# tesseract-robotics/trajopt

Measured on NVIDIA H100. Metric: converged trajectories/sec (7-DOF x 30 wp, batch 1024), higher is better.
Workload: dtype f64

## Files before the change

### trajopt_b200/csrc/kernels.h

```cpp
#pragma once
#include "device_types.cuh"

namespace tb200 {
struct EvalExtra;
struct SolveCtl;
using SolveKernelFn = void (*)(DevProblem, EvalExtra, SolveCtl);
using EvalKernelFn = void (*)(DevProblem, EvalExtra, int, const double*);
SolveKernelFn solve_kernel_for(int D, bool pair_rows, bool sing);
EvalKernelFn eval_kernel_for(int D, bool sing);
int eval_debug_prof(unsigned long long* out, int reset);
constexpr int kQpProfSlots = 32;
int qp_debug_prof(unsigned long long* out, int reset);
}
```

### trajopt_b200/csrc/qp_cta_kernel.cuh

```cuda
#pragma once
#include "device_types.cuh"
#include "joint_terms.cuh"

namespace tb200 {

#ifdef TB200_PROFILE
static __device__ unsigned long long g_prof[32];
#define PROF_T0() const long long prof_t0_ = clock64()
#define PROF_ADD(slot) do { if (q.tid == 0) atomicAdd(&g_prof[slot], (unsigned long long)(clock64() - prof_t0_)); } while (0)
#define PROF_COUNT(slot) do { if (q.tid == 0) atomicAdd(&g_prof[slot], 1ull); } while (0)
#define PROF_ADD2(slot, slot2) do { if (q.tid == 0) { const unsigned long long d_ = clock64() - prof_t0_; \
    atomicAdd(&g_prof[slot], d_); atomicAdd(&g_prof[slot2], d_); } } while (0)
#else
#define PROF_T0()
#define PROF_ADD(slot)
#define PROF_COUNT(slot)
#define PROF_ADD2(slot, slot2)
#endif
#if defined(TB200_PROFILE) && defined(TB200_PROFILE_CHECK)
#define PROF_CHK_T0() long long pc_ = clock64()
#define PROF_CHK(slot) do { const long long n_ = clock64(); if (q.tid == 0) atomicAdd(&g_prof[slot], (unsigned long long)(n_ - pc_)); pc_ = n_; } while (0)
#else
#define PROF_CHK_T0()
#define PROF_CHK(slot)
#endif

constexpr int kQpThreads = 256;
constexpr int kQpThreadsC = 256;
constexpr double kOsqpInf = 1e30;
constexpr double kMinScaling = 1e-4, kMaxScaling = 1e4;
constexpr double kVerifyTol = 1e-9;
constexpr int kVerifyRounds = 3;
constexpr double kRhoMin = 1e-6, kRhoMax = 1e6, kRhoTol = 1e-4, kRhoEqOverIneq = 1e3;
enum { QPS_UNSOLVED = 0, QPS_SOLVED = 1, QPS_SOLVED_INACC = 2, QPS_PINF = 3, QPS_PINF_INACC = 4, QPS_DINF = 5,
       QPS_DINF_INACC = 6, QPS_MAXITER = 7, QPS_NONCVX = 8 };

__device__ __forceinline__ double limit_scaling(double v) {
  v = v < kMinScaling ? 1.0 : v;
  return v > kMaxScaling ? kMaxScaling : v;
}

struct QpSmem {
  int SA, SLM, SU, beta, x, zb, yb, v1, w, qs, lbs, ubs, Dz, v2, Pb, tmp, red, colptr, colent, rints, rows, total, row_cap;
  int factor_smem, pband_smem;
  int pinv;
};

struct PinvPlan {
  int ok;
  int Ns, nS;
  int PR;
  int ZS, HO;
  int WS;
  int SS;
  int zo, wo, so;
  int total;
};
__host__ __device__ inline PinvPlan pinv_plan(int M, int nb) {
  PinvPlan pl;
  pl.Ns = M / 4;
  pl.nS = pl.Ns * nb;
  pl.PR = (M - pl.Ns) * nb;
  const int Np = M * nb, blk = nb * nb;
  pl.ok = (nb % 2 == 0) && nb <= 14 && pl.Ns <= 3 && pl.PR + 2 * pl.nS <= 256;
  pl.ZS = Np + ((4 - Np % 16) + 16) % 16;
  pl.HO = ((Np / 2 + 6) / 16) * 16 + 2;
  if (pl.HO > Np) pl.HO = Np;
  pl.WS = 2 * nb + 2;
  pl.SS = pl.nS + (pl.nS & 1);
  const int fA = (M * blk + 15) & ~15, fL = fA + 8, fU = (M * blk + 1) & ~1;
  const int zn = pl.nS * pl.ZS;
  pl.zo = 0;
  pl.wo = ((zn > fA + fL + fU ? zn : fA + fL + fU) + 15) & ~15;
  pl.so = pl.wo + ((pl.PR * pl.WS + 1) & ~1);
  pl.total = pl.so + pl.nS * pl.SS;
  return pl;
}
constexpr int kQpSmemBudget = 28800;
__host__ __device__ inline int qp_block_count(int N, int nb) { return (N + nb - 1) / nb; }
__host__ __device__ inline int qp_even(int v) { return (v + 1) & ~1; }
__host__ __device__ inline int qp_factor_doubles(int N, int nb) { return 3 * qp_even(qp_block_count(N, nb) * nb * nb); }
__host__ __device__ inline size_t qp_cta_global_doubles(int N, int nb) {
  const PinvPlan pl = pinv_plan(qp_block_count(N, nb), nb);
  return static_cast<size_t>(qp_factor_doubles(N, nb)) + static_cast<size_t>(pl.nS) * pl.ZS;
}
__host__ __device__ inline QpSmem qp_smem_layout(int N, int nb, int row_stride, int CN, int max_rows, bool factor_global) {
  const int M = qp_block_count(N, nb), Np = M * nb, blk = nb * nb;
  QpSmem s;
  int o = 0;
  s.beta = o; o += qp_even(Np);
  s.x = o;    o += qp_even(Np);
  s.zb = o;   o += qp_even(Np);
  s.yb = o;   o += qp_even(Np);
  s.v1 = o;   o += qp_even(Np);
  s.w = o;    o += qp_even(Np);
  s.qs = o;   o += qp_even(Np);
  s.lbs = o;  o += qp_even(Np);
  s.ubs = o;  o += qp_even(Np);
  s.Dz = o;   o += qp_even(Np);
  s.v2 = o;   o += qp_even(Np);
// ... 103 lines not shown
    double v = vals[k];
    if ((SUM_MASK >> k) & 1u) {
#pragma unroll
      for (int off = 16; off > 0; off >>= 1) v += __shfl_xor_sync(0xffffffffu, v, off);
    } else {
      v = warp_max_norm(v);
    }
    vals[k] = v;
  }
  if (lane == 0) {
#pragma unroll
    for (int k = 0; k < NQ; ++k) red[k * 8 + wid] = vals[k];
  }
  __syncthreads();
#pragma unroll
  for (int k = 0; k < NQ; ++k) {
    if ((SUM_MASK >> k) & 1u) {
      double acc = red[k * 8];
#pragma unroll
      for (int w = 1; w < kQpThreads / 32; ++w) acc += red[k * 8 + w];
      vals[k] = acc;
    } else {
      vals[k] = warp_max_norm(red[k * 8 + (lane & 7)]);
    }
  }
  __syncthreads();
}

struct SysW {
  bool polish;
  double sig, rho_aux;
#ifdef TB200_PROFILE
  int prof_kind = 0;
#endif
};

__device__ __forceinline__ int row_var(const int* I, int k) {
  return I[RI_BASE] + min(k, I[RI_CNT] - 1) * I[RI_STRIDE];
}

template <int NB>
__device__ __forceinline__ void load_row(double (&a)[NB], const double* src) {
  const double2* s2 = reinterpret_cast<const double2*>(src);
#pragma unroll
  for (int k = 0; k < NB / 2; ++k) {
    const double2 v = s2[k];
    a[2 * k] = v.x;
    a[2 * k + 1] = v.y;
  }
}
template <int NB>
__device__ __forceinline__ void store_row(double* dst, const double (&a)[NB]) {
  double2* d2 = reinterpret_cast<double2*>(dst);
#pragma unroll
  for (int k = 0; k < NB / 2; ++k) d2[k] = make_double2(a[2 * k], a[2 * k + 1]);
}
template <int NB>
__device__ __forceinline__ void row_times_mat(double (&out)[NB], const double (&x)[NB], const double* Y) {
#pragma unroll
  for (int k = 0; k < NB; ++k) {
    double y[NB];
    load_row<NB>(y, Y + k * NB);
#pragma unroll
    for (int j = 0; j < NB; ++j) out[j] += x[k] * y[j];
  }
}
template <int NB>
__device__ __forceinline__ void row_times_matT(double (&out)[NB], const double (&x)[NB], const double* Y) {
#pragma unroll
  for (int j = 0; j < NB; ++j) {
    double y[NB];
    load_row<NB>(y, Y + j * NB);
    double a0 = 0.0, a1 = 0.0;
#pragma unroll
    for (int k = 0; k < NB; k += 2) {
      a0 += x[k] * y[k];
      a1 += x[k + 1] * y[k + 1];
    }
    out[j] += a0 + a1;
  }
}
template <int NB, bool WARP>
__device__ inline bool bcr_factor(const QpCtx& q) {
  static_assert(!WARP || NB <= 16, "a block per half warp");
  constexpr int BLK = NB * NB, G = kQpThreads / 2;
  constexpr int CH1 = WARP ? kQpThreads / 16 : kQpThreads / NB, CH2 = G / NB;
  extern __shared__ double sm[];
  double* const SA = WARP ? sm + (q.SA - q.smbase) : q.SA;
  double* const SLM = WARP ? sm + (q.SLM - q.smbase) : q.SLM;
  double* const SU = WARP ? sm + (q.SU - q.smbase) : q.SU;
  const int M = q.M, tid = q.tid;
  const int grp = tid >= G, gt = tid - (grp ? G : 0);
  int bad = 0;
  for (int l = 0; (1 << l) - 1 < M; ++l) {
    const int s = 1 << l, first = s - 1, sh = l + 1;
    const int nE = (M + s) >> sh, nS = M >> sh;
    PROF_T0();
    for (int e0 = 0; e0 < nE; e0 += CH1) {
      const int nc = (nE - e0 < CH1) ? nE - e0 : CH1;
      const int e = WARP ? tid >> 4 : tid / NB, i = WARP ? tid & 15 : tid % NB;
      const bool act = WARP ? (i < NB && e < nc) : tid < nc * NB;
      double* A = SA + (first + ((e0 + (act ? e : 0)) << sh)) * BLK + (act ? i : 0) * NB;
      double a[NB];
      load_row<NB>(a, A);
#pragma unroll
      for (int k = 0; k < NB; ++k) {
        double* prow = q.tmp + (k & 1) * (CH1 * NB) + e * NB;
        if (act && i == k) {
          const double piv = a[k];
          if (!(piv > 0.0)) bad = 1;
          const double ip = 1.0 / piv;
#pragma unroll
          for (int j = 0; j < NB; ++j) a[j] = (j == k) ? ip : a[j] * ip;
          store_row<NB>(prow, a);
        }
        if constexpr (WARP) __syncwarp();
        else __syncthreads();
        if (act && i != k) {
          double pr[NB];
          load_row<NB>(pr, prow);
          const double f = a[k];
#pragma unroll
          for (int j = 0; j < NB; ++j) a[j] = (j == k) ? -f * pr[k] : a[j] - f * pr[j];
        }
      }
      if (act) store_row<NB>(A, a);
    }
    __syncthreads();
    PROF_ADD(30);
    for (int e0 = 0; e0 < nE; e0 += CH2) {
      const int nc = (nE - e0 < CH2) ? nE - e0 : CH2;
      const bool act = gt < nc * NB;
      const int e = e0 + (act ? gt / NB : 0), i = gt % NB;
      const int p = first + (e << sh);
      const double* Ai = SA + p * BLK;
      if (act && grp == 0 && p + s < M) {
        double x[NB], out[NB];
        load_row<NB>(x, SLM + (p + s) * BLK + i * NB);
#pragma unroll
        for (int j = 0; j < NB; ++j) out[j] = 0.0;
        row_times_mat<NB>(out, x, Ai);
        store_row<NB>(SU + p * BLK + i * NB, out);
      }
      if (act && grp == 1 && p - s >= 0) {
        double x[NB], out[NB];
        const double* L = SLM + p * BLK + i;
#pragma unroll
        for (int k = 0; k < NB; ++k) x[k] = L[k * NB];
#pragma unroll
        for (int j = 0; j < NB; ++j) out[j] = 0.0;
        row_times_mat<NB>(out, x, Ai);
        store_row<NB>(SU + (p - s) * BLK + i * NB, out);
      }
    }
    __syncthreads();
    for (int e0 = 0; e0 < nS; e0 += CH2) {
      const int nc = (nS - e0 < CH2) ? nS - e0 : CH2;
      const bool act = gt < nc * NB;
      const int e = e0 + (act ? gt / NB : 0), i = gt % NB;
      const int j = first + s + (e << sh), p = j - s;
      double keep[NB];
#pragma unroll
      for (int c = 0; c < NB; ++c) keep[c] = 0.0;
      if (act && grp == 0) {
        double x[NB], t1[NB];
        load_row<NB>(x, SU + p * BLK + i * NB);
#pragma unroll
        for (int c = 0; c < NB; ++c) t1[c] = 0.0;
        row_times_matT<NB>(t1, x, SLM + j * BLK);
        if (p - s >= 0) row_times_mat<NB>(keep, x, SLM + p * BLK);
        double arow[NB];
        load_row<NB>(arow, SA + j * BLK + i * NB);
#pragma unroll
        for (int c = 0; c < NB; ++c) arow[c] -= t1[c];
        store_row<NB>(SA + j * BLK + i * NB, arow);
      }
      if (act && grp == 1 && j + s < M) {
        double x[NB];
        load_row<NB>(x, SU + j * BLK + i * NB);
        row_times_mat<NB>(keep, x, SLM + (j + s) * BLK);
      }
      __syncthreads();
      if (act && grp == 0) {
#pragma unroll
        for (int c = 0; c < NB; ++c) keep[c] = -keep[c];
        store_row<NB>(SLM + j * BLK + i * NB, keep);
      }
      if (act && grp == 1 && j + s < M) {
        double arow[NB];
        load_row<NB>(arow, SA + j * BLK + i * NB);
#pragma unroll
        for (int c = 0; c < NB; ++c) arow[c] -= keep[c];
        store_row<NB>(SA + j * BLK + i * NB, arow);
      }
    }
    __syncthreads();
    for (int t = tid; t < nE * BLK; t += kQpThreads) {
      const int e = t / BLK, r = t % BLK;
      const int p = first + (e << sh);
      if (p - s >= 0) SLM[p * BLK + r] = SU[(p - s) * BLK + r];
    }
    __syncthreads();
  }
  if (tid == 0) q.flag[0] = 0.0;
  __syncthreads();
  if (bad) q.flag[0] = 1.0;
  __syncthreads();
  const bool ok = q.flag[0] == 0.0;
  __syncthreads();
  return ok;
}

template <int NB>
__device__ __forceinline__ double dot_row(const double* __restrict__ m, const double* __restrict__ v) {
  const double2* m2 = reinterpret_cast<const double2*>(m);
  const double2* v2 = reinterpret_cast<const double2*>(v);
  double a0 = 0.0, a1 = 0.0;
#pragma unroll
  for (int k = 0; k < NB / 2; ++k) {
    const double2 mm = m2[k], vv = v2[k];
    a0 += mm.x * vv.x;
    a1 += mm.y * vv.y;
  }
  return a0 + a1;
}
template <int NB>
__device__ inline void bcr_solve(const QpCtx& q, double* v, double* w) {
  constexpr int BLK = NB * NB, H = NB / 2;
  const int M = q.M, tid = q.tid, side = tid & 1, task0 = tid >> 1;
  __syncthreads();
  int l = 0;
  for (; (2 << l) - 1 < M; ++l) {
    const int s = 1 << l, sh = l + 1, nS = M >> sh;
    for (int tb = 0; tb < nS * NB; tb += kQpThreads / 2) {
      if (tb + ((tid & ~31) >> 1) >= nS * NB) continue;
      const int task = tb + task0;
      const int e = task / NB, r = task % NB;
      const bool act = e < nS;
      const int j = 2 * s - 1 + ((act ? e : 0) << sh);
      const int pb = side ? j + s : j - s;
      const bool valid = act && pb < M;
      const int pbc = valid ? pb : j - s;
      const double* mat = (side ? q.SLM : q.SU) + pbc * BLK + r * NB;
      double a = dot_row<NB>(mat, v + pbc * NB);
      a = valid ? a : 0.0;
      const double o = __shfl_xor_sync(0xffffffffu, a, 1);
      if (act && side == 0) v[j * NB + r] -= a + o;
    }
    __syncthreads();
  }
  for (; l >= 0; --l) {
    const int s = 1 << l, first = s - 1, sh = l + 1;
    if (first >= M) continue;
    const int nE = (M + s) >> sh;
    for (int tb = 0; tb < nE * NB; tb += kQpThreads / 2) {
      if (tb + ((tid & ~31) >> 1) >= nE * NB) continue;
      const int task = tb + task0;
      const int e = task / NB, r = task % NB;
      const bool act = e < nE;
      const int p = first + ((act ? e : 0) << sh);
      const bool hasl = p - s >= 0, hasr = p + s < M;
      const double* X = (side ? q.SU : q.SA) + p * BLK + r;
      const double* y = side ? w + (hasr ? p + s : 0) * NB : v + p * NB;
      const double* Um = q.SLM + p * BLK + (side ? H * NB : 0) + r;
      const double* wl = w + (hasl ? p - s : 0) * NB + (side ? H : 0);
      double a0 = 0.0, a1 = 0.0, a2 = 0.0;
#pragma unroll
      for (int k = 0; k < NB; k += 2) {
        a0 += X[k * NB] * y[k];
        a1 += X[(k + 1) * NB] * y[k + 1];
      }
#pragma unroll
      for (int k = 0; k < H; ++k) a2 += Um[k * NB] * wl[k];
      const double dx = a0 + a1;
      const double acc = (side ? (hasr ? -dx : 0.0) : dx) - (hasl ? a2 : 0.0);
      const double o = __shfl_xor_sync(0xffffffffu, acc, 1);
      if (act && side == 0) w[p * NB + r] = acc + o;
    }
    __syncthreads();
  }
}

struct SolveRoles {
  int n_fwd, n_lvl;
  int f0_warps, b0_warps;
// ... 364 lines not shown
  for (int k = 0; k < 2; ++k) {
    const double da = fmin(F[R_DYA0 + k], 0.0);
    a[0] = fmax(a[0], fabs(F[R_EA0 + k] * da));
    a[2] = fmax(a[2], fabs((F[R_U0 + k] * d + F[R_B0 + k] * da) / F[R_DA0 + k]));
  }
  return d;
}
__device__ __forceinline__ void pinf_var_terms(const double ratio, const double ub, const double lb, const double d,
                                               double (&a)[3]) {
  a[0] = fmax(a[0], fabs(ratio * d));
  a[1] += ub * fmax(d, 0.0) + lb * fmin(d, 0.0);
}
__device__ __forceinline__ void dinf_row_terms(const double* F, double (&a)[2]) {
#pragma unroll
  for (int k = 0; k < 2; ++k) {
    a[0] = fmax(a[0], fabs(F[R_DA0 + k] * F[R_DXA0 + k]));
    a[1] += F[R_QA0 + k] * F[R_DXA0 + k];
  }
}
__device__ __forceinline__ unsigned long long guess_mix(unsigned long long v) {
  v += 0x9e3779b97f4a7c15ull;
  v = (v ^ (v >> 30)) * 0xbf58476d1ce4e5b9ull;
  v = (v ^ (v >> 27)) * 0x94d049bb133111ebull;
  return v ^ (v >> 31);
}
__device__ __forceinline__ unsigned long long guess_row_hash(const double* F, const int* I, const int r, const int nrows,
                                                             const int N) {
  unsigned long long h = 0ull;
  const unsigned long long mc = static_cast<unsigned long long>(nrows);
  if (F[R_Z] - F[R_LO] < -F[R_Y]) h += guess_mix(2ull * r);
  else if (F[R_UP] - F[R_Z] < F[R_Y]) h += guess_mix(2ull * r + 1ull);
  for (int k = 0; k < I[RI_AUX]; ++k) {
    const unsigned long long idx = mc + N + I[RI_PAD] + k;
    if (F[R_ZA0 + k] - 0.0 < -F[R_YA0 + k]) h += guess_mix(2ull * idx);
    else if (kOsqpInf * F[R_EA0 + k] - F[R_ZA0 + k] < F[R_YA0 + k]) h += guess_mix(2ull * idx + 1ull);
  }
  return h;
}
__device__ __forceinline__ unsigned long long guess_var_hash(const double zb, const double yb, const double lb,
                                                             const double ub, const int i, const int nrows) {
  const unsigned long long idx = static_cast<unsigned long long>(nrows) + i;
  if (zb - lb < -yb) return guess_mix(2ull * idx);
  if (ub - zb < yb) return guess_mix(2ull * idx + 1ull);
  return 0ull;
}
enum ChkQ { CHK_PA0 = 14, CHK_PA1, CHK_PA2, CHK_DA0, CHK_DA1, kChkHash };
constexpr unsigned kChkSumMask = (1u << CHK_PA1) | (1u << CHK_DA1);

__device__ inline void rows_prepare_weights(const QpCtx& q, const SysW& w) {
  for (int r = q.tid; r < q.nrows; r += kQpThreads) {
    double* F = q.F(r);
    const int naux = q.I(r)[RI_AUX];
    const double Wr = w.polish ? fabs(F[R_PW]) : ((F[R_RHO] != 0.0) ? q.rho_eq : q.rho);
    const double wa0 = w.polish ? fabs(F[R_PWA0]) : w.rho_aux;
    const double wa1 = w.polish ? fabs(F[R_PWA1]) : w.rho_aux;
    const double g0 = (naux >= 1) ? w.sig + wa0 * F[R_B0] * F[R_B0] : 1.0;
    const double g1 = (naux == 2) ? w.sig + wa1 * F[R_B1] * F[R_B1] : 1.0;
    const double den = g0 * g1 + Wr * (F[R_U0] * F[R_U0] * g1 + F[R_U1] * F[R_U1] * g0);
    F[R_WRR] = Wr;
    F[R_G0] = g0;
    F[R_G1] = g1;
    F[R_DEN] = den;
    F[R_IDEN] = 1.0 / den;
    F[R_IWRR] = (Wr != 0.0) ? 1.0 / Wr : 0.0;
    F[R_WR] = Wr * g0 * g1 / den;
  }
  __syncthreads();
}
__device__ __forceinline__ double xbound_weight(const QpCtx& q, const SysW& w, int j) {
  const double adm = (q.ubs[j] - q.lbs[j] < kRhoTol) ? q.rho_eq : q.rho;
  return w.polish ? fabs(q.zb[j]) : adm;
}

__device__ __forceinline__ double pivot_rcp(const double x) {
  double r;
  asm("rcp.approx.ftz.f64 %0, %1;" : "=d"(r) : "d"(x));
  double e = fma(-x, r, 1.0);
  r = fma(r, e, r);
  e = fma(-x, r, 1.0);
  r = fma(r, e, r);
  e = fma(-x, r, 1.0);
  return fma(r, e, r);
}
template <int QN>
__device__ __forceinline__ bool gj_rows(double (&a)[QN], double diag, const bool active, const int mat, const int row,
                                        const int n, const int n_max, double* tmp, const int nmat, const int bar) {
  constexpr int BS = QN + 2;
  double* const csv = tmp + 2 * nmat * BS + mat * QN;
  bool bad = false;
  double pv_mine = pivot_rcp(diag), my_cs = 1.0, rs = 1.0, inv_rs = 1.0;
#pragma unroll 1
  for (int k = 0; k < n_max; ++k) {
    double* buf = tmp + ((k & 1) * nmat + mat) * BS;
    const bool piv = active && row == k;
    if (piv) {
      bad |= !(diag > 0.0);
#pragma unroll
      for (int j = 0; j < QN; j += 2) *reinterpret_cast<double2*>(buf + j) = make_double2(a[j], a[j + 1]);
      buf[k] = 0.0;
      buf[QN] = pv_mine;
      my_cs = -pv_mine;
      csv[k] = my_cs;
      rs = pv_mine;
      inv_rs = diag;
      diag = pv_mine;
    }
    asm volatile("bar.sync %0, 64;" ::"r"(bar) : "memory");
    if (active && k < n && !piv) {
      const double tr = buf[row];
      const bool ahead = row > k;
      const double f = ahead ? tr : -tr * my_cs;
      const double g = f * buf[QN];
      diag = ahead ? diag - g * f : diag + g * f;
      const double gs = g * inv_rs;
#pragma unroll
      for (int j = 0; j < QN; j += 2) {
        const double2 t = *reinterpret_cast<const double2*>(buf + j);
        a[j] -= gs * t.x;
        a[j + 1] -= gs * t.y;
      }
      if (ahead) pv_mine = pivot_rcp(diag);
    }
  }
  if (active) {
#pragma unroll
    for (int j = 0; j < QN; ++j) a[j] = (j == row) ? diag : ((j < n) ? a[j] * (rs * csv[j]) : 0.0);
  }
  return bad;
}

template <int NB>
__device__ inline bool pinv_factor(const QpCtx& q) {
  constexpr int QN = 3 * NB, blk = NB * NB;
  static_assert(QN % 2 == 0, "pivot rows move as double2");
  static_assert(QN <= 64, "a partition on two warps");
  extern __shared__ double sm[];
  const int tid = q.tid, M = q.M, Np = q.Np;
  const int PR = q.pl.PR, nS = q.pl.nS, Ns = q.pl.Ns, ZS = q.pl.ZS, WS = q.pl.WS, SS = q.pl.SS;
  double* const fbase = sm + (q.SA - q.smbase);
  const double* const SA = fbase;
  const double* const SLM = sm + (q.SLM - q.smbase);
  double* const Z = fbase + q.pl.zo;
  double* const W = fbase + q.pl.wo;
  double* const S = fbase + q.pl.so;
  double* const tmp = q.tmp.ptr();
  const int nparts = (M + 3) / 4;
  bool bad = false;
#ifdef TB200_PROFILE
  long long pf_ = clock64();
#define PROF_PF(slot) do { const long long n_ = clock64(); if (tid == 0) atomicAdd(&g_prof[slot], (unsigned long long)(n_ - pf_)); pf_ = n_; } while (0)
#else
#define PROF_PF(slot)
#endif
  {
    const int p = tid >> 6, lr = tid & 63, pr = p * QN + lr;
    const bool part = p < nparts;
    const int npb = !part ? 0 : (M - 4 * p) < 3 ? (M - 4 * p) : 3;
    const bool prow = lr < npb * NB;
    const int kb = lr / NB, r = lr % NB, gb = 4 * p + kb;
    double a[QN];
#pragma unroll
    for (int j = 0; j < QN; ++j) {
      const int cb = j / NB, c = j % NB;
      double v = 0.0;
      if (prow && cb < npb) {
        if (cb == kb) v = SA[gb * blk + r * NB + c];
        else if (cb == kb - 1) v = SLM[gb * blk + r * NB + c];
        else if (cb == kb + 1) v = SLM[(gb + 1) * blk + c * NB + r];
      }
      a[j] = v;
    }
    PROF_PF(0);
    const double dg = prow ? SA[gb * blk + r * NB + r] : 1.0;
    if (part) bad |= gj_rows<QN>(a, dg, prow, p, lr, npb * NB, (M < 3 ? M : 3) * NB, tmp, nparts, 1 + p);
    PROF_PF(4);
    if (prow) {
#pragma unroll
      for (int j = 0; j < QN; ++j) q.pi_g[j * PR + pr] = a[j];
      const bool has_l = p > 0, has_r = 4 * p + 3 < M;
#pragma unroll 2
      for (int j = 0; j < NB; ++j) {
        double wl = 0.0, wr = 0.0;
        if (has_l) {
#pragma unroll
          for (int c = 0; c < NB; ++c) wl += a[c] * SLM[(4 * p) * blk + c * NB + j];
        }
        if (has_r) {
#pragma unroll
          for (int c = 0; c < NB; ++c) wr += a[2 * NB + c] * SLM[(4 * p + 3) * blk + j * NB + c];
        }
        W[pr * WS + j] = wl;
        W[pr * WS + NB + j] = wr;
      }
    }
  }
  __syncthreads();
  for (int e = tid; e < nS * nS; e += kQpThreads) {
    const int ra = e / nS, ca = e % nS, sa = ra / NB, i = ra % NB, sb = ca / NB, j = ca % NB;
    double v = 0.0;
    if (sa == sb || sb == sa + 1 || sb == sa - 1) {
      const bool use_l = sb <= sa, use_r = sb >= sa && 4 * sa + 4 < M;
      const double* cl = SLM + (4 * sa + 3) * blk + i * NB;
      const double* wl = W + (sa * QN + 2 * NB) * WS + (sb == sa ? NB : 0) + j;
      const double* cr = SLM + (4 * sa + 4) * blk + i;
      const double* wr = W + ((sa + 1) * QN) * WS + (sb == sa ? 0 : NB) + j;
      double s0 = 0.0, s1 = 0.0, s2 = 0.0, s3 = 0.0;
      if (use_l) {
#pragma unroll
        for (int rr = 0; rr < NB; rr += 2) {
          s0 += cl[rr] * wl[rr * WS];
          s1 += cl[rr + 1] * wl[(rr + 1) * WS];
        }
      }
      if (use_r) {
#pragma unroll
        for (int rr = 0; rr < NB; rr += 2) {
          s2 += cr[rr * NB] * wr[rr * WS];
          s3 += cr[(rr + 1) * NB] * wr[(rr + 1) * WS];
        }
      }
      v = ((sa == sb) ? SA[(4 * sa + 3) * blk + i * NB + j] : 0.0) - ((s0 + s1) + (s2 + s3));
    }
    S[ra * SS + ca] = v;
  }
  __syncthreads();
  PROF_PF(14);
  {
    const bool srow = tid < nS;
    double a[QN];
#pragma unroll
    for (int j = 0; j < QN; ++j) a[j] = (srow && j < nS) ? S[tid * SS + j] : 0.0;
    const double dg = srow ? S[tid * SS + tid] : 1.0;
    if (tid < 64) bad |= gj_rows<QN>(a, dg, srow, 0, tid, nS, nS, tmp, 1, 1);
    if (srow) {
#pragma unroll
      for (int j = 0; j < QN; ++j)
        if (j < nS) S[tid * SS + j] = a[j];
    }
  }
  __syncthreads();
  PROF_PF(15);
  if (tid < Np) {
    const int col = tid, cb = col / NB, c = col % NB, p = cb / 4;
    if (cb % 4 == 3) {
      for (int sr = 0; sr < nS; ++sr) Z[sr * ZS + col] = S[sr * SS + p * NB + c];
    } else {
      const bool has_l = p > 0, has_r = 4 * p + 3 < M;
      const double* wrow = W + (p * QN + (cb % 4) * NB + c) * WS;
      double wv[2 * NB];
#pragma unroll
      for (int t = 0; t < 2 * NB; ++t) wv[t] = wrow[t];
      const double* sl = S + (has_l ? (p - 1) * NB : 0);
      const double* sr_ = S + (has_r ? p * NB : 0);
#pragma unroll 2
      for (int sr = 0; sr < nS; ++sr) {
        double s0 = 0.0, s1 = 0.0, s2 = 0.0, s3 = 0.0;
#pragma unroll
        for (int t = 0; t < NB; t += 2) {
          s0 += sl[sr * SS + t] * wv[t];
          s1 += sl[sr * SS + t + 1] * wv[t + 1];
          s2 += sr_[sr * SS + t] * wv[NB + t];
          s3 += sr_[sr * SS + t + 1] * wv[NB + t + 1];
        }
        Z[sr * ZS + col] = -((s0 + s1) + (s2 + s3));
      }
    }
  }
  (void)Ns;
  const bool ok = !__syncthreads_or(bad ? 1 : 0);
  PROF_PF(9);
  return ok;
}

template <int NB, bool PINV, bool WARP>
__device__ __noinline__ bool assemble_factor(const QpCtx& q, const SysW& w) {
  PROF_T0();
  rows_prepare_weights(q, w);
  constexpr int nb = NB, blk = NB * NB;
  extern __shared__ double sm[];
  constexpr bool SMEM = PINV || WARP;
  double* const SA = SMEM ? sm + (q.SA - q.smbase) : q.SA;
  double* const SLM = SMEM ? sm + (q.SLM - q.smbase) : q.SLM;
  const int N = q.N, HB = 2 * q.D, PW = HB + 1, CN = q.CN;
  for (int t = q.tid; t < q.M * blk; t += kQpThreads) {
    SA[t] = 0.0;
    SLM[t] = 0.0;
  }
  __syncthreads();
  for (int i = q.tid; i < q.Np; i += kQpThreads) {
    const int p = i / nb, r = i % nb;
    double* Arow = SA + static_cast<size_t>(p) * blk + r * nb;
    double* Lrow = SLM + static_cast<size_t>(p) * blk + r * nb;
    if (i >= N) {
      Arow[r] = 1.0;
      continue;
    }
    auto add = [&](int k, double val) {
      if (k <= r) Arow[r - k] = __dadd_rn(Arow[r - k], val);
      else Lrow[nb + r - k] = __dadd_rn(Lrow[nb + r - k], val);
    };
    for (int t = 0; t < q.n_band; ++t) {
      const int k = q.band_offs[t];
      if (k <= i) add(k, q.c * q.Dz[i] * q.Pband[i * PW + k] * q.Dz[i - k]);
    }
    add(0, w.sig + xbound_weight(q, w, i) * q.beta[i] * q.beta[i]);
    for (int e = q.colptr[i]; e < q.colptr[i + 1]; ++e) {
      const int ent = q.colent[e], rw = ent >> 5, k = ent & 31;
      const double* R = q.R(rw);
      const double wr = R[2 * CN + R_WR];
      if (wr == 0.0) continue;
      const int stride = q.I(rw)[RI_STRIDE];
      const double* as = R + CN;
      const double ai = wr * as[k];
      for (int k2 = 0; k2 <= k; ++k2) add((k - k2) * stride, ai * as[k2]);
    }
  }
  __syncthreads();
  for (int t = q.tid; t < q.M * blk; t += kQpThreads) {
    const int p = t / blk, i = (t % blk) / nb, j = t % nb;
    if (j > i) SA[static_cast<size_t>(p) * blk + i * nb + j] = SA[static_cast<size_t>(p) * blk + j * nb + i];
  }
  __syncthreads();
#ifdef TB200_PROFILE
  const int pk = w.polish ? 2 : w.prof_kind;
  if (pk == 1) PROF_COUNT(31);
#endif
  PROF_ADD2(10, 24 + 2 * pk);
  bool ok;
  {
    PROF_T0();
    if constexpr (PINV) ok = pinv_factor<NB>(q);
    else ok = bcr_factor<NB, WARP>(q);
    PROF_ADD2(11, 25 + 2 * pk);
  }
  return ok;
}

struct QpPlan {
  bool use_reg, use_pinv, fuse, fast_polish;
};
__host__ __device__ inline QpPlan qp_plan(bool regok, int pinv, int rows_smem, int M, int nb, bool fast_passes) {
  QpPlan pl;
  pl.use_reg = regok && solve_roles_fit(M, nb);
  pl.use_pinv = regok && pinv && rows_smem;
  pl.fuse = pl.use_pinv && fast_passes;
  pl.fast_polish = pl.use_pinv && fast_passes && M * nb <= kQpThreads && solve_roles_fit(M, nb);
  return pl;
}
enum QpPath {
  QPP_BLOCK_PINV = 1 << 0,
  QPP_BLOCK_FAST = 1 << 1,
  QPP_BLOCK_GENERIC = 1 << 2,
  QPP_BLOCK_SOA = 1 << 3,
  QPP_FACTOR_GLOBAL = 1 << 4,
  QPP_BAND_GLOBAL = 1 << 5,
  QPP_ROWS_GLOBAL = 1 << 6,
  QPP_FUSED_CHECK = 1 << 7,
  QPP_POLISH_FAST = 1 << 8,
  QPP_POLISH_GENERIC = 1 << 9
};
__host__ __device__ inline int qp_plan_block(const QpPlan& pl, int rows_smem) {
  if (pl.use_pinv) return QPP_BLOCK_PINV;
  if (!rows_smem) return QPP_BLOCK_SOA;
  return pl.use_reg ? QPP_BLOCK_FAST : QPP_BLOCK_GENERIC;
}

struct QpOut {
  int status, iters, polish;
  double rho;
  double pri_res, dua_res, pol_pri, pol_dua, c;
  int pol_factor_ok, rho_updates, rounds;
};

template <int CN, class Base>
__device__ __forceinline__ void scatter_columns(const QpCtx& q, Base base) {
  for (int i = q.tid; i < q.Np; i += kQpThreads) {
    double s = 0.0;
    if (i < q.N) {
      s = base(i);
      for (int e = q.colptr[i]; e < q.colptr[i + 1]; ++e) {
        const int ent = q.colent[e], r = ent >> 5, k = ent & 31;
        const double* R = q.R(r);
        s += R[CN + k] * R[2 * CN + R_COEF];
      }
    }
    q.v1[i] = s;
  }
  __syncthreads();
}
template <int CN>
__device__ __forceinline__ double row_dot(const QpCtx& q, const double* R, const int* I, const double* v) {
  double z = 0.0;
  const int base = I[RI_BASE], stride = I[RI_STRIDE], last = I[RI_CNT] - 1;
#pragma unroll
  for (int k = 0; k < CN; ++k) z += R[CN + k] * v[base + min(k, last) * stride];
  return z;
}
__device__ __forceinline__ void row_backsub(const double* F, double zeta, double& a0, double& a1) {
  const double Wr = F[R_WRR], ra0 = F[R_RA0], ra1 = F[R_RA1], u0 = F[R_U0], u1 = F[R_U1];
  const double iden = F[R_IDEN];
  a0 = (F[R_G1] * (ra0 - Wr * u0 * zeta) + Wr * u1 * (u1 * ra0 - u0 * ra1)) * iden;
  a1 = (F[R_G0] * (ra1 - Wr * u1 * zeta) + Wr * u0 * (u0 * ra1 - u1 * ra0)) * iden;
}
__device__ __forceinline__ double row_reduce_coef(const double* F, double ra0, double ra1, double zcoef) {
  return zcoef - F[R_WRR] * (F[R_U0] * ra0 * F[R_G1] + F[R_U1] * ra1 * F[R_G0]) * F[R_IDEN];
}
template <int CNc>
__device__ __forceinline__ void admm_row_entry(const double* R, double* F, const double& sigma, const double& rho_aux) {
  const double s = F[R_WRR] * F[R_Z] - F[R_Y];
  const double ra0 = sigma * F[R_XA0] - F[R_QA0] + F[R_U0] * s + F[R_B0] * (rho_aux * F[R_ZA0] - F[R_YA0]);
  const double ra1 = sigma * F[R_XA1] - F[R_QA1] + F[R_U1] * s + F[R_B1] * (rho_aux * F[R_ZA1] - F[R_YA1]);
  F[R_RA0] = ra0;
  F[R_RA1] = ra1;
  const double cf = row_reduce_coef(F, ra0, ra1, s);
// ... 881 lines not shown
template <int NB, int PAIR, bool REGOK>
__device__ inline QpOut qp_solve_block(QpCtx& q, const QpSettings& st, bool warm, double warm_rho,
                                       const double* ws_x, const double* ws_yb, const bool fast_passes) {
  constexpr int CNc = PAIR ? ((NB > 3) ? NB : 3) : ((NB / 2 > 3) ? NB / 2 : 3);
  const int N = q.N, tid = q.tid;
  QpOut out{QPS_UNSOLVED, 0, 0, st.rho, 0, 0, 0, 0, 0, -1, 0, 0};
  double rho;
  double eps_scale;
  int iter, round;
  q.sigma = st.sigma;
  q.alpha = st.alpha;
  {
    rho = warm ? warm_rho : st.rho;
    rho = fmin(fmax(rho, kRhoMin), kRhoMax);
    eps_scale = 1.0;
    iter = 0;
    round = 0;
    q.rho = rho;
    q.rho_eq = kRhoEqOverIneq * rho;
    if (warm) {
      for (int i = tid; i < q.Np; i += kQpThreads) {
        if (i < N) {
          q.x[i] = ws_x[i] / q.Dz[i];
          q.yb[i] = ws_yb[i] * q.Dz[i] / q.beta[i] * q.c;
          q.zb[i] = q.beta[i] * q.x[i];
        } else {
          q.x[i] = q.yb[i] = q.zb[i] = 0.0;
        }
      }
      __syncthreads();
      for (int r = tid; r < q.nrows; r += kQpThreads) {
        double* R = q.R(r);
        double* F = q.F(r);
        const int naux = q.I(r)[RI_AUX];
        F[R_XA0] = (naux >= 1) ? F[R_XA0] / F[R_DA0] : 0.0;
        F[R_XA1] = (naux == 2) ? F[R_XA1] / F[R_DA1] : 0.0;
        F[R_Y] = F[R_Y] / F[R_E] * q.c;
        F[R_YA0] = (naux >= 1) ? F[R_YA0] / F[R_EA0] * q.c : 0.0;
        F[R_YA1] = (naux == 2) ? F[R_YA1] / F[R_EA1] * q.c : 0.0;
        F[R_Z] = row_dot<CNc>(q, R, q.I(r), q.x) + F[R_U0] * F[R_XA0] + F[R_U1] * F[R_XA1];
        F[R_ZA0] = F[R_B0] * F[R_XA0];
        F[R_ZA1] = F[R_B1] * F[R_XA1];
      }
    } else {
      for (int i = tid; i < q.Np; i += kQpThreads) q.x[i] = q.zb[i] = q.yb[i] = 0.0;
      for (int r = tid; r < q.nrows; r += kQpThreads) {
        double* F = q.F(r);
        F[R_XA0] = F[R_XA1] = F[R_Z] = F[R_Y] = F[R_ZA0] = F[R_ZA1] = F[R_YA0] = F[R_YA1] = 0.0;
      }
    }
    __syncthreads();
  }
  SysW sysw{false, st.sigma, rho};
  bool factor_ok = true;

  const QpPlan plan = qp_plan(REGOK, q.pinv, q.rows_smem, q.M, NB, fast_passes);
  const bool use_reg = plan.use_reg;
  const bool use_pinv = plan.use_pinv;
  using BlockFn = void (*)(const QpCtx&, double, int, int);
  const bool fuse = plan.fuse;
  const bool fast_polish = plan.fast_polish;
  bool fused_chk = false;
  auto run_block = [&](int n, bool keep_last) {
    fused_chk = fuse && keep_last;
    if constexpr (REGOK) {
      if (use_pinv || use_reg) {
        BlockFn volatile fn = use_pinv ? &admm_block_pinv<NB, PAIR>
                                       : (q.rows_smem ? &admm_block_fast<NB, PAIR> : &admm_block_soa<NB, PAIR>);
        fn(q, sysw.rho_aux, n, keep_last ? (fuse ? 2 : 1) : 0);
        return;
      }
    }
    BlockFn volatile fn = q.rows_smem ? &admm_block<NB, PAIR> : &admm_block_soa<NB, PAIR>;
    fn(q, sysw.rho_aux, n, keep_last ? 1 : 0);
  };
  using FactorFn = bool (*)(const QpCtx&, const SysW&);
  auto factorize = [&](const SysW& wts) -> bool {
    fused_chk = false;
    FactorFn f = &assemble_factor<NB, false, false>;
    if constexpr (NB <= 16) {
      if (fast_passes && __isShared(q.SA)) f = &assemble_factor<NB, false, true>;
    }
    if constexpr (REGOK) {
      if (use_pinv && !wts.polish) f = &assemble_factor<NB, true, false>;
    }
    FactorFn volatile fn = f;
    return fn(q, wts);
  };
  auto stash_z = [&](const bool restore) {
    extern __shared__ double sm[];
    double2* zs = reinterpret_cast<double2*>(sm + (q.SA - q.smbase) + q.pl.zo);
    double2* zg = reinterpret_cast<double2*>(q.z_stash);
    const int n2 = q.pl.nS * q.pl.ZS / 2;
    if (restore) for (int i = tid; i < n2; i += kQpThreads) zs[i] = zg[i];
    else for (int i = tid; i < n2; i += kQpThreads) zg[i] = zs[i];
    __syncthreads();
    if (restore) rows_prepare_weights(q, sysw);
  };
  { PROF_T0(); factor_ok = factorize(sysw); PROF_ADD(6); }
#ifdef TB200_PROFILE
  sysw.prof_kind = 1;
#endif

  double* dxs = q.scratch;
  double* dyb = q.scratch + q.Np;
  double* st_x = q.scratch + 2 * q.Np;
  double* st_zb = q.scratch + 3 * q.Np;
  double* st_yb = q.scratch + 4 * q.Np;
  double pri_res = 0.0, dua_res = 0.0;
  int status = factor_ok ? QPS_UNSOLVED : QPS_NONCVX;
  bool early_verified = false;
  unsigned long long prev_guess = 0ull, failed_guess = 0ull, pending_guess = 0ull;
  bool have_prev_guess = false, have_failed_guess = false;
  double n_z = 0, n_ax = 0, n_q = 0, n_aty = 0, n_px = 0, s_pri = 0, s_dua = 0, s_z = 0, s_ax = 0, s_q = 0, s_aty = 0, s_px = 0;

  auto info_pass = [&](const bool scaled) {
    PROF_CHK_T0();
    p_matvec<NB>(q, q.x, q.v2);
    PROF_CHK(4);
    double m[14] = {0, 0, 0, 0, 0, 0, 0, 0, 0, 0, 0, 0, 0, 0};
    for (int r = tid; r < q.nrows; r += kQpThreads) {
      const double* R = q.R(r);
      double* F = q.F(r);
      const double ax = row_dot<CNc>(q, R, q.I(r), q.x) + F[R_U0] * F[R_XA0] + F[R_U1] * F[R_XA1];
      info_row_terms(F, ax, m);
      F[R_COEF] = F[R_Y];
    }
    __syncthreads();
    PROF_CHK(14);
    scatter_columns<CNc>(q, [&](int i) { return q.beta[i] * q.yb[i]; });
    for (int i = tid; i < N; i += kQpThreads)
      info_var_terms(q.Dz[i], q.beta[i], q.x[i], q.zb[i], q.v1[i], q.v2[i], q.qs[i], m);
    if (scaled) {
      block_reduce<14, 0u>(q, m);
      s_pri = m[7]; s_z = m[8]; s_ax = m[9]; s_dua = m[10]; s_aty = m[11]; s_q = m[12]; s_px = m[13];
    } else {
      double m7[7] = {m[0], m[1], m[2], m[3], m[4], m[5], m[6]};
      block_reduce<7, 0u>(q, m7);
#pragma unroll
      for (int k = 0; k < 7; ++k) m[k] = m7[k];
    }
    PROF_CHK(15);
    pri_res = m[0];
    dua_res = m[3] * q.cinv;
    n_z = m[1]; n_ax = m[2]; n_aty = m[4]; n_q = m[5]; n_px = m[6];
  };

  auto fused_q = [&](const int k) -> double {
    extern __shared__ double sm[];
    const double* const chk = sm + (q.tmp - q.smbase) + k * 8;
    if ((kChkSumMask >> k) & 1u) {
      double acc = chk[0];
      for (int w = 1; w < kQpThreads / 32; ++w) acc += chk[w];
      return acc;
    }
    return warp_max_norm(chk[tid & 7]);
  };
  auto residuals = [&](const bool scaled) {
    if (!fused_chk) {
      info_pass(scaled);
      return;
    }
    double m[14];
#pragma unroll
    for (int k = 0; k < 14; ++k) m[k] = (k < 7 || scaled) ? fused_q(k) : 0.0;
    pri_res = m[0];
    dua_res = m[3] * q.cinv;
// ... 807 lines not shown
```

Before: 1465.

## Split factorization row work across more lanes in BCR and pinv separator solve

In the warp-mode block cyclic reduction, the Schur-update phase now gives each warp one separator block, with each row split across two lanes, and synchronises with __syncwarp instead of block-wide barriers. The pinv separator Gauss-Jordan solve can split each row across three threads on four warps when fast passes are enabled. The assembly step writes the upper triangle of each block directly instead of running a separate symmetrisation pass. The aim is to use more threads and fewer block barriers in the small dense factorizations. The cost is more complex indexing, more barrier participants in the GJ solve, and an added even-NB requirement for warp mode.

```diff
diff --git a/trajopt_b200/csrc/kernels.h b/trajopt_b200/csrc/kernels.h
--- a/trajopt_b200/csrc/kernels.h
+++ b/trajopt_b200/csrc/kernels.h
@@ -9,6 +9,6 @@
 SolveKernelFn solve_kernel_for(int D, bool pair_rows, bool sing);
 EvalKernelFn eval_kernel_for(int D, bool sing);
 int eval_debug_prof(unsigned long long* out, int reset);
-constexpr int kQpProfSlots = 32;
+constexpr int kQpProfSlots = 40;
 int qp_debug_prof(unsigned long long* out, int reset);
 }
diff --git a/trajopt_b200/csrc/qp_cta_kernel.cuh b/trajopt_b200/csrc/qp_cta_kernel.cuh
--- a/trajopt_b200/csrc/qp_cta_kernel.cuh
+++ b/trajopt_b200/csrc/qp_cta_kernel.cuh
@@ -5,17 +5,21 @@
 namespace tb200 {
 
 #ifdef TB200_PROFILE
-static __device__ unsigned long long g_prof[32];
+static __device__ unsigned long long g_prof[40];
 #define PROF_T0() const long long prof_t0_ = clock64()
 #define PROF_ADD(slot) do { if (q.tid == 0) atomicAdd(&g_prof[slot], (unsigned long long)(clock64() - prof_t0_)); } while (0)
 #define PROF_COUNT(slot) do { if (q.tid == 0) atomicAdd(&g_prof[slot], 1ull); } while (0)
 #define PROF_ADD2(slot, slot2) do { if (q.tid == 0) { const unsigned long long d_ = clock64() - prof_t0_; \
     atomicAdd(&g_prof[slot], d_); atomicAdd(&g_prof[slot2], d_); } } while (0)
+#define PROF_MARK_T0() long long prof_m_ = clock64()
+#define PROF_MARK(slot) do { const long long n_ = clock64(); if (q.tid == 0) atomicAdd(&g_prof[slot], (unsigned long long)(n_ - prof_m_)); prof_m_ = n_; } while (0)
 #else
 #define PROF_T0()
 #define PROF_ADD(slot)
 #define PROF_COUNT(slot)
 #define PROF_ADD2(slot, slot2)
+#define PROF_MARK_T0()
+#define PROF_MARK(slot)
 #endif
 #if defined(TB200_PROFILE) && defined(TB200_PROFILE_CHECK)
 #define PROF_CHK_T0() long long pc_ = clock64()
@@ -285,8 +289,8 @@
 }
 template <int NB, bool WARP>
 __device__ inline bool bcr_factor(const QpCtx& q) {
-  static_assert(!WARP || NB <= 16, "a block per half warp");
-  constexpr int BLK = NB * NB, G = kQpThreads / 2;
+  static_assert(!WARP || (NB <= 16 && NB % 2 == 0), "a block per half warp, a survivor row on two lanes");
+  constexpr int BLK = NB * NB, G = kQpThreads / 2, H = NB / 2;
   constexpr int CH1 = WARP ? kQpThreads / 16 : kQpThreads / NB, CH2 = G / NB;
   extern __shared__ double sm[];
   double* const SA = WARP ? sm + (q.SA - q.smbase) : q.SA;
@@ -331,6 +335,7 @@
     }
     __syncthreads();
     PROF_ADD(30);
+    PROF_MARK_T0();
     for (int e0 = 0; e0 < nE; e0 += CH2) {
       const int nc = (nE - e0 < CH2) ? nE - e0 : CH2;
       const bool act = gt < nc * NB;
@@ -357,44 +362,102 @@
       }
     }
     __syncthreads();
-    for (int e0 = 0; e0 < nS; e0 += CH2) {
-      const int nc = (nS - e0 < CH2) ? nS - e0 : CH2;
-      const bool act = gt < nc * NB;
-      const int e = e0 + (act ? gt / NB : 0), i = gt % NB;
-      const int j = first + s + (e << sh), p = j - s;
-      double keep[NB];
-#pragma unroll
-      for (int c = 0; c < NB; ++c) keep[c] = 0.0;
-      if (act && grp == 0) {
-        double x[NB], t1[NB];
-        load_row<NB>(x, SU + p * BLK + i * NB);
-#pragma unroll
-        for (int c = 0; c < NB; ++c) t1[c] = 0.0;
-        row_times_matT<NB>(t1, x, SLM + j * BLK);
-        if (p - s >= 0) row_times_mat<NB>(keep, x, SLM + p * BLK);
-        double arow[NB];
-        load_row<NB>(arow, SA + j * BLK + i * NB);
-#pragma unroll
-        for (int c = 0; c < NB; ++c) arow[c] -= t1[c];
-        store_row<NB>(SA + j * BLK + i * NB, arow);
-      }
-      if (act && grp == 1 && j + s < M) {
-        double x[NB];
-        load_row<NB>(x, SU + j * BLK + i * NB);
-        row_times_mat<NB>(keep, x, SLM + (j + s) * BLK);
-      }
-      __syncthreads();
-      if (act && grp == 0) {
-#pragma unroll
-        for (int c = 0; c < NB; ++c) keep[c] = -keep[c];
-        store_row<NB>(SLM + j * BLK + i * NB, keep);
-      }
-      if (act && grp == 1 && j + s < M) {
-        double arow[NB];
-        load_row<NB>(arow, SA + j * BLK + i * NB);
-#pragma unroll
-        for (int c = 0; c < NB; ++c) arow[c] -= keep[c];
-        store_row<NB>(SA + j * BLK + i * NB, arow);
+    PROF_MARK(37);
+    if constexpr (WARP) {
+      const int w = tid >> 5, lane = tid & 31, i = lane >> 1, c0 = (lane & 1) * H;
+      const bool act = i < NB;
+      const int ir = act ? i : 0;
+      for (int e0 = 0; e0 < nS; e0 += kQpThreads / 32) {
+        if (e0 + w >= nS) continue;
+        const int j = first + s + ((e0 + w) << sh), p = j - s;
+        double x[NB], t1[H], keep[H], arow[H];
+        load_row<NB>(x, SU + p * BLK + ir * NB);
+        const double* Lj = SLM + j * BLK;
+#pragma unroll
+        for (int c = 0; c < H; ++c) {
+          double y[NB];
+          load_row<NB>(y, Lj + (c0 + c) * NB);
+          double a0 = 0.0, a1 = 0.0;
+#pragma unroll
+          for (int k = 0; k < NB; k += 2) {
+            a0 += x[k] * y[k];
+            a1 += x[k + 1] * y[k + 1];
+          }
+          t1[c] = 0.0;
+          t1[c] += a0 + a1;
+        }
+#pragma unroll
+        for (int c = 0; c < H; ++c) keep[c] = 0.0;
+        if (p - s >= 0) {
+#pragma unroll
+          for (int k = 0; k < NB; ++k) {
+#pragma unroll
+            for (int c = 0; c < H; ++c) keep[c] += x[k] * SLM[p * BLK + k * NB + c0 + c];
+          }
+        }
+        double* Aj = SA + j * BLK + ir * NB + c0;
+#pragma unroll
+        for (int c = 0; c < H; ++c) arow[c] = Aj[c] - t1[c];
+        const bool hasr = j + s < M;
+        if (hasr) {
+          load_row<NB>(x, SU + j * BLK + ir * NB);
+#pragma unroll
+          for (int c = 0; c < H; ++c) t1[c] = 0.0;
+#pragma unroll
+          for (int k = 0; k < NB; ++k) {
+#pragma unroll
+            for (int c = 0; c < H; ++c) t1[c] += x[k] * SLM[(j + s) * BLK + k * NB + c0 + c];
+          }
+        }
+        __syncwarp();
+        if (act) {
+#pragma unroll
+          for (int c = 0; c < H; ++c) {
+            SLM[j * BLK + i * NB + c0 + c] = -keep[c];
+            Aj[c] = hasr ? arow[c] - t1[c] : arow[c];
+          }
+        }
+      }
+    } else {
+      for (int e0 = 0; e0 < nS; e0 += CH2) {
+        const int nc = (nS - e0 < CH2) ? nS - e0 : CH2;
+        const bool act = gt < nc * NB;
+        const int e = e0 + (act ? gt / NB : 0), i = gt % NB;
+        const int j = first + s + (e << sh), p = j - s;
+        double keep[NB];
+#pragma unroll
+        for (int c = 0; c < NB; ++c) keep[c] = 0.0;
+        if (act && grp == 0) {
+          double x[NB], t1[NB];
+          load_row<NB>(x, SU + p * BLK + i * NB);
+#pragma unroll
+          for (int c = 0; c < NB; ++c) t1[c] = 0.0;
+          row_times_matT<NB>(t1, x, SLM + j * BLK);
+          if (p - s >= 0) row_times_mat<NB>(keep, x, SLM + p * BLK);
+          double arow[NB];
+          load_row<NB>(arow, SA + j * BLK + i * NB);
+#pragma unroll
+          for (int c = 0; c < NB; ++c) arow[c] -= t1[c];
+          store_row<NB>(SA + j * BLK + i * NB, arow);
+        }
+        if (act && grp == 1 && j + s < M) {
+          double x[NB];
+          load_row<NB>(x, SU + j * BLK + i * NB);
+          row_times_mat<NB>(keep, x, SLM + (j + s) * BLK);
+        }
+        __syncthreads();
+        if (act && grp == 0) {
+#pragma unroll
+          for (int c = 0; c < NB; ++c) keep[c] = -keep[c];
+          store_row<NB>(SLM + j * BLK + i * NB, keep);
+        }
+        if (act && grp == 1 && j + s < M) {
+          double arow[NB];
+          load_row<NB>(arow, SA + j * BLK + i * NB);
+#pragma unroll
+          for (int c = 0; c < NB; ++c) arow[c] -= keep[c];
+          store_row<NB>(SA + j * BLK + i * NB, arow);
+        }
       }
     }
     __syncthreads();
@@ -404,6 +467,7 @@
       if (p - s >= 0) SLM[p * BLK + r] = SU[(p - s) * BLK + r];
     }
     __syncthreads();
+    PROF_MARK(38);
   }
   if (tid == 0) q.flag[0] = 0.0;
   __syncthreads();
@@ -934,10 +998,14 @@
   e = fma(-x, r, 1.0);
   return fma(r, e, r);
 }
-template <int QN>
-__device__ __forceinline__ bool gj_rows(double (&a)[QN], double diag, const bool active, const int mat, const int row,
-                                        const int n, const int n_max, double* tmp, const int nmat, const int bar) {
+template <int QN, int C = 1, int NT = 64>
+__device__ __forceinline__ bool gj_rows(double (&a)[QN / C], double diag, const bool active, const int mat, const int row,
+                                        const int part, const int n, const int n_max, double* tmp, const int nmat,
+                                        const int bar) {
   constexpr int BS = QN + 2;
+  constexpr int QW = QN / C;
+  static_assert(QN % C == 0 && QW % 2 == 0, "the shares of a pivot row move as double2");
+  const int c0 = part * QW;
   double* const csv = tmp + 2 * nmat * BS + mat * QN;
   bool bad = false;
   double pv_mine = pivot_rcp(diag), my_cs = 1.0, rs = 1.0, inv_rs = 1.0;
@@ -948,16 +1016,18 @@
     if (piv) {
       bad |= !(diag > 0.0);
 #pragma unroll
-      for (int j = 0; j < QN; j += 2) *reinterpret_cast<double2*>(buf + j) = make_double2(a[j], a[j + 1]);
-      buf[k] = 0.0;
-      buf[QN] = pv_mine;
+      for (int j = 0; j < QW; j += 2) *reinterpret_cast<double2*>(buf + c0 + j) = make_double2(a[j], a[j + 1]);
+      if (k >= c0 && k < c0 + QW) buf[k] = 0.0;
       my_cs = -pv_mine;
-      csv[k] = my_cs;
+      if (part == 0) {
+        buf[QN] = pv_mine;
+        csv[k] = my_cs;
+      }
       rs = pv_mine;
       inv_rs = diag;
       diag = pv_mine;
     }
-    asm volatile("bar.sync %0, 64;" ::"r"(bar) : "memory");
+    asm volatile("bar.sync %0, %1;" ::"r"(bar), "n"(NT) : "memory");
     if (active && k < n && !piv) {
       const double tr = buf[row];
       const bool ahead = row > k;
@@ -966,8 +1036,8 @@
       diag = ahead ? diag - g * f : diag + g * f;
       const double gs = g * inv_rs;
 #pragma unroll
-      for (int j = 0; j < QN; j += 2) {
-        const double2 t = *reinterpret_cast<const double2*>(buf + j);
+      for (int j = 0; j < QW; j += 2) {
+        const double2 t = *reinterpret_cast<const double2*>(buf + c0 + j);
         a[j] -= gs * t.x;
         a[j + 1] -= gs * t.y;
       }
@@ -976,16 +1046,17 @@
   }
   if (active) {
 #pragma unroll
-    for (int j = 0; j < QN; ++j) a[j] = (j == row) ? diag : ((j < n) ? a[j] * (rs * csv[j]) : 0.0);
+    for (int j = 0; j < QW; ++j) a[j] = (c0 + j == row) ? diag : ((c0 + j < n) ? a[j] * (rs * csv[c0 + j]) : 0.0);
   }
   return bad;
 }
 
-template <int NB>
+template <int NB, bool SPLIT>
 __device__ inline bool pinv_factor(const QpCtx& q) {
   constexpr int QN = 3 * NB, blk = NB * NB;
   static_assert(QN % 2 == 0, "pivot rows move as double2");
   static_assert(QN <= 64, "a partition on two warps");
+  static_assert(!SPLIT || 3 * QN <= 128, "the separator rows on four warps");
   extern __shared__ double sm[];
   const int tid = q.tid, M = q.M, Np = q.Np;
   const int PR = q.pl.PR, nS = q.pl.nS, Ns = q.pl.Ns, ZS = q.pl.ZS, WS = q.pl.WS, SS = q.pl.SS;
@@ -1022,10 +1093,10 @@
       }
       a[j] = v;
     }
-    PROF_PF(0);
+    PROF_PF(32);
     const double dg = prow ? SA[gb * blk + r * NB + r] : 1.0;
-    if (part) bad |= gj_rows<QN>(a, dg, prow, p, lr, npb * NB, (M < 3 ? M : 3) * NB, tmp, nparts, 1 + p);
-    PROF_PF(4);
+    if (part) bad |= gj_rows<QN>(a, dg, prow, p, lr, 0, npb * NB, (M < 3 ? M : 3) * NB, tmp, nparts, 1 + p);
+    PROF_PF(33);
     if (prow) {
 #pragma unroll
       for (int j = 0; j < QN; ++j) q.pi_g[j * PR + pr] = a[j];
@@ -1076,22 +1147,24 @@
     S[ra * SS + ca] = v;
   }
   __syncthreads();
-  PROF_PF(14);
+  PROF_PF(34);
   {
-    const bool srow = tid < nS;
-    double a[QN];
-#pragma unroll
-    for (int j = 0; j < QN; ++j) a[j] = (srow && j < nS) ? S[tid * SS + j] : 0.0;
-    const double dg = srow ? S[tid * SS + tid] : 1.0;
-    if (tid < 64) bad |= gj_rows<QN>(a, dg, srow, 0, tid, nS, nS, tmp, 1, 1);
+    constexpr int C = SPLIT ? 3 : 1, QW = QN / C, NT = SPLIT ? 128 : 64;
+    const int row = tid / C, part = tid % C;
+    const bool srow = row < nS;
+    double a[QW];
+#pragma unroll
+    for (int j = 0; j < QW; ++j) a[j] = (srow && part * QW + j < nS) ? S[row * SS + part * QW + j] : 0.0;
+    const double dg = srow ? S[row * SS + row] : 1.0;
+    if (tid < NT) bad |= gj_rows<QN, C, NT>(a, dg, srow, 0, row, part, nS, nS, tmp, 1, 1);
     if (srow) {
 #pragma unroll
-      for (int j = 0; j < QN; ++j)
-        if (j < nS) S[tid * SS + j] = a[j];
-    }
-  }
-  __syncthreads();
-  PROF_PF(15);
+      for (int j = 0; j < QW; ++j)
+        if (part * QW + j < nS) S[row * SS + part * QW + j] = a[j];
+    }
+  }
+  __syncthreads();
+  PROF_PF(35);
   if (tid < Np) {
     const int col = tid, cb = col / NB, c = col % NB, p = cb / 4;
     if (cb % 4 == 3) {
@@ -1120,7 +1193,7 @@
   }
   (void)Ns;
   const bool ok = !__syncthreads_or(bad ? 1 : 0);
-  PROF_PF(9);
+  PROF_PF(36);
   return ok;
 }
 
@@ -1166,11 +1239,7 @@
       const double ai = wr * as[k];
       for (int k2 = 0; k2 <= k; ++k2) add((k - k2) * stride, ai * as[k2]);
     }
-  }
-  __syncthreads();
-  for (int t = q.tid; t < q.M * blk; t += kQpThreads) {
-    const int p = t / blk, i = (t % blk) / nb, j = t % nb;
-    if (j > i) SA[static_cast<size_t>(p) * blk + i * nb + j] = SA[static_cast<size_t>(p) * blk + j * nb + i];
+    for (int c = 0; c < r; ++c) SA[static_cast<size_t>(p) * blk + c * nb + r] = Arow[c];
   }
   __syncthreads();
 #ifdef TB200_PROFILE
@@ -1181,7 +1250,7 @@
   bool ok;
   {
     PROF_T0();
-    if constexpr (PINV) ok = pinv_factor<NB>(q);
+    if constexpr (PINV) ok = pinv_factor<NB, WARP>(q);
     else ok = bcr_factor<NB, WARP>(q);
     PROF_ADD2(11, 25 + 2 * pk);
   }
@@ -2229,7 +2298,7 @@
       if (fast_passes && __isShared(q.SA)) f = &assemble_factor<NB, false, true>;
     }
     if constexpr (REGOK) {
-      if (use_pinv && !wts.polish) f = &assemble_factor<NB, true, false>;
+      if (use_pinv && !wts.polish) f = fast_passes ? &assemble_factor<NB, true, true> : &assemble_factor<NB, true, false>;
     }
     FactorFn volatile fn = f;
     return fn(q, wts);
```

New measurement: 1484, median of 6. +1.3%, better.
